# HudsonAlpha/rust-msbwt

Measured on AMD Instinct MI355X. Metric: k-mer count queries/sec (whole node), higher is better.
Workload: dtype u64

## Files before the change

rust-msbwt_amd/_build.py:

```python
import os
import subprocess
import sys

HERE = os.path.dirname(os.path.abspath(__file__))
CSRC = os.path.join(HERE, "csrc")
LIB = os.path.join(HERE, "libmsbwt_hip.so")
SOURCES = ["capi.cpp", "index_build.cpp", "query.cpp", "sources.cpp", "spectrum.cpp", "produce.cpp", "multi_device.cpp", "kernels.hip", "lanes.hip", "lanes_tier.hip", "lanes_wide.hip", "lanes_xwide.hip", "extend.hip", "sparse_table.hip", "device_build.hip", "pair_index.hip", "gather.hip", "order.hip", "run_build.hip", "reads_build.hip", "run_encode.hip", "merge.hip", "merge_many.hip", "source_index.hip", "spectrum.hip", "plane_index.cpp", "run_index.cpp", "npy_io.cpp", "rle_codec.cpp"]
HEADERS = ["handle.hpp", "index_build.hpp", "kernels.hpp", "lanes_kernel.hpp", "sparse_table.hpp", "sparse_build.hpp", "sparse_policy.hpp", "device_build.hpp", "pair_index.hpp", "gather.hpp", "order.hpp", "run_build.hpp", "reads_build.hpp", "run_encode.hpp", "merge.hpp", "merge_common.hpp", "source_index.hpp", "frontier.hpp", "spectrum.hpp", "rank_ops.hpp", "search_common.hpp", "host_pipeline.hpp", "plane_index.hpp", "run_index.hpp", "table_policy.hpp", "npy_io.hpp", "rle_codec.hpp", os.path.join("..", "..", "include", "msbwt_hip.h")]


def hipcc():
    for cand in (os.environ.get("HIPCC"), "/opt/rocm/bin/hipcc", "hipcc"):
        if cand and (os.path.isabs(cand) and os.path.exists(cand) or not os.path.isabs(cand)):
            return cand
    return "hipcc"


def stale():
    if not os.path.exists(LIB):
        return True
    t = os.path.getmtime(LIB)
    deps = [os.path.join(CSRC, f) for f in SOURCES + HEADERS] + [os.path.abspath(__file__)]
    return any(os.path.getmtime(d) > t for d in deps)


def build(force=False, verbose=False):
    if not force and not stale():
        return LIB
    from concurrent.futures import ThreadPoolExecutor

    objdir = os.path.join(HERE, "build")
    os.makedirs(objdir, exist_ok=True)
    common = ["-O3", "-std=c++17", "-fPIC", "-Wall", "-Wextra"]
    newest_header = max(os.path.getmtime(os.path.join(CSRC, f)) for f in HEADERS)
    newest_header = max(newest_header, os.path.getmtime(os.path.abspath(__file__)))

    def compile_one(src):
        obj = os.path.join(objdir, src + ".o")
        path = os.path.join(CSRC, src)
        if not force and os.path.exists(obj) and os.path.getmtime(obj) > max(os.path.getmtime(path), newest_header):
            return obj
# ... 21 lines not shown
```

rust-msbwt_amd/csrc/host_pipeline.hpp:

```cpp
#pragma once
#include <hip/hip_runtime_api.h>

#include <algorithm>
#include <condition_variable>
#include <cstdint>
#include <cstring>
#include <functional>
#include <memory>
#include <mutex>
#include <thread>
#include <vector>

namespace msbwt {

class CopyPool {
  public:
    explicit CopyPool(int threads) {
        for (int t = 0; t < threads; ++t) workers_.emplace_back([this, t] { loop(t); });
    }
    ~CopyPool() {
        {
            std::lock_guard<std::mutex> lock(mu_);
            stop_ = true;
        }
        wake_.notify_all();
        for (auto &w : workers_) w.join();
    }
    int threads() const { return int(workers_.size()); }

    void copy(void *dst, const void *src, size_t bytes) {
        if (bytes < (size_t(1) << 20) || workers_.empty()) {
            std::memcpy(dst, src, bytes);
            return;
        }
        std::unique_lock<std::mutex> lock(mu_);
        dst_ = static_cast<char *>(dst);
        src_ = static_cast<const char *>(src);
        bytes_ = bytes;
        pending_ = int(workers_.size());
        ++generation_;
        wake_.notify_all();
        done_.wait(lock, [this] { return pending_ == 0; });
    }

  private:
    void loop(int t) {
        uint64_t seen = 0;
        for (;;) {
            std::unique_lock<std::mutex> lock(mu_);
            wake_.wait(lock, [&] { return stop_ || generation_ != seen; });
            if (stop_) return;
            seen = generation_;
            const size_t n = workers_.size(), piece = (bytes_ / n + 63) / 64 * 64;
            const size_t lo = std::min(bytes_, piece * size_t(t)), hi = (size_t(t) + 1 == n) ? bytes_ : std::min(bytes_, lo + piece);
            char *d = dst_;
            const char *s = src_;
            lock.unlock();
            if (hi > lo) std::memcpy(d + lo, s + lo, hi - lo);
            lock.lock();
            if (--pending_ == 0) done_.notify_all();
        }
    }
    std::vector<std::thread> workers_;
    std::mutex mu_;
    std::condition_variable wake_, done_;
    bool stop_ = false;
    uint64_t generation_ = 0;
    int pending_ = 0;
    char *dst_ = nullptr;
    const char *src_ = nullptr;
    size_t bytes_ = 0;
};

struct HostArray {
    const void *in = nullptr;
    void *out = nullptr;
    size_t item_bytes = 0;
};

class HostPipeline {
  public:
    static constexpr int kSlots = 3;
    ~HostPipeline() { release(); }

    using Launch = std::function<hipError_t(size_t, size_t, void *const *, void *const *, hipStream_t)>;

    hipError_t run(size_t n, size_t chunk, const std::vector<HostArray> &ins, const std::vector<HostArray> &outs,
                   hipStream_t compute, const Launch &launch) {
        if (n == 0) return hipSuccess;
        chunk = std::max<size_t>(1, std::min(chunk, n));
        size_t in_bytes = 0, out_bytes = 0;
        std::vector<size_t> in_off, out_off;
        for (const HostArray &a : ins) { in_off.push_back(in_bytes); in_bytes += (chunk * a.item_bytes + 255) / 256 * 256; }
        for (const HostArray &a : outs) { out_off.push_back(out_bytes); out_bytes += (chunk * a.item_bytes + 255) / 256 * 256; }
        hipError_t e = ensure(in_bytes, out_bytes);
        if (e != hipSuccess) return e;
        if (!pool_) {
            const unsigned hw = std::thread::hardware_concurrency();
            pool_.reset(new CopyPool(int(std::max(2u, std::min(hw ? hw / 2 : 4u, 12u)))));
        }
        const size_t nchunks = (n + chunk - 1) / chunk;
        std::vector<void *> d_in(ins.size()), d_out(outs.size());
        auto finish = [&](size_t c) -> hipError_t {
            Slot &s = slots_[c % kSlots];
            hipError_t err = hipEventSynchronize(s.d2h);
            if (err != hipSuccess) return err;
            const size_t first = c * chunk, m = std::min(chunk, n - first);
            for (size_t a = 0; a < outs.size(); ++a)
                pool_->copy(static_cast<char *>(outs[a].out) + first * outs[a].item_bytes, s.h_out + out_off[a], m * outs[a].item_bytes);
            return hipSuccess;
        };
        for (size_t c = 0; c < nchunks + kSlots - 1; ++c) {
            if (c < nchunks) {
                Slot &s = slots_[c % kSlots];
                const size_t first = c * chunk, m = std::min(chunk, n - first);
                for (size_t a = 0; a < ins.size(); ++a)
                    pool_->copy(s.h_in + in_off[a], static_cast<const char *>(ins[a].in) + first * ins[a].item_bytes, m * ins[a].item_bytes);
                for (size_t a = 0; a < ins.size(); ++a) {
                    e = hipMemcpyAsync(s.d_in + in_off[a], s.h_in + in_off[a], m * ins[a].item_bytes, hipMemcpyHostToDevice, h2d_);
                    if (e != hipSuccess) return e;
                    d_in[a] = s.d_in + in_off[a];
                }
                for (size_t a = 0; a < outs.size(); ++a) d_out[a] = s.d_out + out_off[a];
                if ((e = hipEventRecord(s.up, h2d_)) != hipSuccess) return e;
                if ((e = hipStreamWaitEvent(compute, s.up, 0)) != hipSuccess) return e;
                if ((e = launch(first, m, d_in.data(), d_out.data(), compute)) != hipSuccess) return e;
                if ((e = hipEventRecord(s.done, compute)) != hipSuccess) return e;
                if ((e = hipStreamWaitEvent(d2h_, s.done, 0)) != hipSuccess) return e;
                for (size_t a = 0; a < outs.size(); ++a) {
                    e = hipMemcpyAsync(s.h_out + out_off[a], s.d_out + out_off[a], m * outs[a].item_bytes, hipMemcpyDeviceToHost, d2h_);
                    if (e != hipSuccess) return e;
                }
                if ((e = hipEventRecord(s.d2h, d2h_)) != hipSuccess) return e;
            }
            if (c >= size_t(kSlots - 1) && (e = finish(c - (kSlots - 1))) != hipSuccess) return e;
        }
        return hipSuccess;
    }

    void release() {
        for (Slot &s : slots_) {
            if (s.h_in) (void)hipHostFree(s.h_in);
            if (s.h_out) (void)hipHostFree(s.h_out);
            if (s.d_in) (void)hipFree(s.d_in);
            if (s.d_out) (void)hipFree(s.d_out);
            if (s.up) (void)hipEventDestroy(s.up);
            if (s.done) (void)hipEventDestroy(s.done);
            if (s.d2h) (void)hipEventDestroy(s.d2h);
            s = Slot{};
        }
        if (h2d_) (void)hipStreamDestroy(h2d_);
        if (d2h_) (void)hipStreamDestroy(d2h_);
        h2d_ = d2h_ = nullptr;
        in_cap_ = out_cap_ = 0;
    }

  private:
    struct Slot {
        char *h_in = nullptr, *h_out = nullptr, *d_in = nullptr, *d_out = nullptr;
        hipEvent_t up = nullptr, done = nullptr, d2h = nullptr;
    };

    hipError_t ensure(size_t in_bytes, size_t out_bytes) {
        hipError_t e;
        if (!h2d_ && (e = hipStreamCreateWithFlags(&h2d_, hipStreamNonBlocking)) != hipSuccess) return e;
        if (!d2h_ && (e = hipStreamCreateWithFlags(&d2h_, hipStreamNonBlocking)) != hipSuccess) return e;
        for (Slot &s : slots_) {
            if (!s.up && (e = hipEventCreateWithFlags(&s.up, hipEventDisableTiming)) != hipSuccess) return e;
            if (!s.done && (e = hipEventCreateWithFlags(&s.done, hipEventDisableTiming)) != hipSuccess) return e;
            if (!s.d2h && (e = hipEventCreateWithFlags(&s.d2h, hipEventDisableTiming)) != hipSuccess) return e;
        }
        if (in_bytes > in_cap_) {
            for (Slot &s : slots_) {
                if (s.h_in) (void)hipHostFree(s.h_in);
                if (s.d_in) (void)hipFree(s.d_in);
                s.h_in = s.d_in = nullptr;
            }
            in_cap_ = 0;
            for (Slot &s : slots_) {
                if ((e = hipHostMalloc(reinterpret_cast<void **>(&s.h_in), in_bytes, hipHostMallocDefault)) != hipSuccess) return e;
                if ((e = hipMalloc(reinterpret_cast<void **>(&s.d_in), in_bytes)) != hipSuccess) return e;
            }
            in_cap_ = in_bytes;
        }
        if (out_bytes > out_cap_) {
            for (Slot &s : slots_) {
                if (s.h_out) (void)hipHostFree(s.h_out);
                if (s.d_out) (void)hipFree(s.d_out);
                s.h_out = s.d_out = nullptr;
            }
            out_cap_ = 0;
            for (Slot &s : slots_) {
                if ((e = hipHostMalloc(reinterpret_cast<void **>(&s.h_out), out_bytes, hipHostMallocDefault)) != hipSuccess) return e;
                if ((e = hipMalloc(reinterpret_cast<void **>(&s.d_out), out_bytes)) != hipSuccess) return e;
            }
            out_cap_ = out_bytes;
        }
        return hipSuccess;
    }

    Slot slots_[kSlots];
    hipStream_t h2d_ = nullptr, d2h_ = nullptr;
    size_t in_cap_ = 0, out_cap_ = 0;
    std::unique_ptr<CopyPool> pool_;
};

}
```

rust-msbwt_amd/csrc/query.cpp:

```cpp
#include <algorithm>
#include <atomic>
#include <chrono>
#include <cstring>
#include <string>
#include <vector>

#include "gather.hpp"
#include "handle.hpp"
#include "order.hpp"

namespace {

constexpr size_t kMailQueries = 64, kMailKmerBytes = 4096;
constexpr size_t kMailDone = 0;
constexpr size_t kMailKmers = 64, kMailCounts = kMailKmers + kMailKmerBytes, kMailSyms = kMailCounts + 8 * kMailQueries,
                 kMailL = kMailSyms + 64, kMailH = kMailL + 8 * kMailQueries, kMailOutL = kMailH + 8 * kMailQueries,
                 kMailOutH = kMailOutL + 8 * kMailQueries, kMailBytes = kMailOutH + 8 * kMailQueries;

int ensure_mail(msbwt_rle *h) {
    if (int rc = ensure_runtime(h)) return rc;
    if (h->mail) return MSBWT_OK;
    void *host = nullptr, *dev = nullptr;
    HIP_TRY(h, hipHostMalloc(&host, kMailBytes, hipHostMallocMapped | hipHostMallocCoherent));
    const hipError_t e = hipHostGetDevicePointer(&dev, host, 0);
    if (e != hipSuccess) {
        (void)hipHostFree(host);
        return hip_fail(h, e, "hipHostGetDevicePointer");
    }
    std::memset(host, 0, kMailBytes);
    h->mail = static_cast<uint8_t *>(host);
    h->d_mail = static_cast<uint8_t *>(dev);
    return MSBWT_OK;
}

bool order_pays(msbwt_rle *h, const IndexView &v, size_t k, size_t n) {
    if (h->wanted_order <= 0 || v.block_format != kBlocksPlanes || v.pair_blocks == nullptr) return false;
    return k >= 12 && k <= 64 && n >= 4096 && n <= 0xFFFFFFFFull && lanes_serves(v, uint32_t(k));
}

bool ensure_order_scratch(msbwt_rle::TicketSlot &slot, size_t bytes) {
    if (bytes <= slot.order_bytes) return true;
    if (slot.order_scratch) (void)hipFree(slot.order_scratch);
// ... 106 lines not shown
            if (!ensure_range_scratch(slot, std::min(n, kBySourcePiece) * 2 * sizeof(uint64_t))) return hipErrorOutOfMemory;
            uint64_t *pairs = static_cast<uint64_t *>(slot.range_scratch);
            const SourceView sv = h->sources.view(v.total);
            hipError_t e = hipSuccess;
            for (size_t first = 0; first < n && e == hipSuccess; first += kBySourcePiece) {
                const size_t m = std::min(kBySourcePiece, n - first);
                e = launch_kmer_ranges(v, d_kmers + first * k, uint32_t(k), m, pairs, pairs + 1, 2u, h->d_flags + which, stream);
                if (e == hipSuccess) e = launch_range_sources(sv, pairs, pairs + 1, 2u, m, d_out + first * sv.n_sources, h->d_flags + which, stream);
            }
            return e;
        });
    });
}

int launch_sources_of_ranges(msbwt_rle *h, const uint64_t *d_l, const uint64_t *d_h, size_t n, uint64_t *d_out, hipStream_t stream, int which) {
    return timed_launch(h, stream, [&] { return launch_range_sources(h->sources.view(h->totals.total), d_l, d_h, 1u, n, d_out, h->d_flags + which, stream); });
}

int need_sources(msbwt_rle *h) { return h->sources.n_sources ? int(MSBWT_OK) : fail(h, MSBWT_ERR_NOT_LOADED, "no sources attached"); }

size_t by_source_chunk(const msbwt_rle *h) { return std::min(size_t(1) << 21, (size_t(96) << 20) / (h->sources.n_sources * sizeof(uint64_t))); }

int launch_read_kmers_locked(msbwt_rle *h, const void *d_reads, size_t read_len, size_t n_reads, size_t k,
                                    int ascii, void *d_out_fwd, void *d_out_rc, hipStream_t stream, int which) {
    return timed_with_tickets(h, stream, [&](const IndexView &v) {
        return launch_count_read_kmers(v, static_cast<const uint8_t *>(d_reads), uint32_t(read_len), n_reads, uint32_t(k), ascii != 0,
                                       static_cast<uint64_t *>(d_out_fwd), static_cast<uint64_t *>(d_out_rc), h->d_flags + which, stream);
    });
}

HostArray host_in(const void *p, size_t item_bytes) { return HostArray{p, nullptr, item_bytes}; }
HostArray host_out(void *p, size_t item_bytes) { return HostArray{nullptr, p, item_bytes}; }

template <class Launch>
int run_host_batch(msbwt_rle *h, size_t n, size_t chunk, const std::vector<HostArray> &ins, const std::vector<HostArray> &outs, const char *what,
                   Launch &&launch) {
    int launch_rc = MSBWT_OK;
    const hipError_t e = h->pipe.run(n, chunk, ins, outs, h->stream, [&](size_t, size_t m, void *const *d_in, void *const *d_out, hipStream_t stream) {
        launch_rc = launch(m, d_in, d_out, stream);
        return launch_rc ? hipErrorUnknown : hipSuccess;
    });
    if (launch_rc) return launch_rc;
    if (e != hipSuccess) return hip_fail(h, e, (std::string(what) + " pipeline").c_str());
    return status_of(h, h->stream, kHostFlags);
}

template <class Launch, class CopyOut>
int mailbox_call(msbwt_rle *h, IndexView &v, bool poll, Launch &&launch, CopyOut &&copy_out) {
    volatile uint64_t *done = reinterpret_cast<volatile uint64_t *>(h->mail + kMailDone);
    const uint64_t seq = ++h->mail_seq;
    if (poll) {
        v.done = reinterpret_cast<uint64_t *>(h->d_mail + kMailDone);
        v.done_seq = seq;
    }
    if (int rc = launch()) return rc;
    bool seen = false;
    if (poll) {
        const auto give_up = std::chrono::steady_clock::now() + std::chrono::milliseconds(2);
        for (unsigned spins = 0; !(seen = *done == seq); ++spins)
            if ((spins & 1023u) == 1023u && std::chrono::steady_clock::now() > give_up) break;
    }
    if (!seen) HIP_TRY(h, hipStreamSynchronize(h->stream));
    std::atomic_thread_fence(std::memory_order_acquire);
    return copy_out() ? status_of(h, h->stream, kHostFlags) : MSBWT_OK;
}

// ... 6 lines not shown
    Call c(ch);
    if (int rc = c.open(n && (!d_out_counts || (!d_kmers && k)), "null device pointer")) return rc;
    return launch_count(c.h, static_cast<const uint8_t *>(d_kmers), k, n, static_cast<uint64_t *>(d_out_counts),
                        static_cast<hipStream_t>(hip_stream), kDeviceFlags);
}

int msbwt_rle_count_kmers_packed_device(const msbwt_rle *ch, const void *d_kmers2bit, size_t k, size_t n, void *d_out_counts, void *hip_stream) {
    Call c(ch);
    if (int rc = c.open(n && (!d_out_counts || !d_kmers2bit), "null device pointer")) return rc;
    if (n == 0) return MSBWT_OK;
    return launch_count_2bit(c.h, static_cast<const uint64_t *>(d_kmers2bit), k, n, static_cast<uint64_t *>(d_out_counts), static_cast<hipStream_t>(hip_stream),
                             kDeviceFlags);
}

int msbwt_rle_count_kmers_packed(const msbwt_rle *ch, const uint64_t *kmers2bit, size_t k, size_t n, void *out_counts, int count_bits) {
    Call c(ch);
    const bool bad_k = k < 1 || k > 64 || (count_bits != 64 && count_bits != 32);
    if (int rc = c.open(bad_k || (n && (!out_counts || !kmers2bit)), bad_k ? "packed queries need 1 <= k <= 64 and 64- or 32-bit counts" : "null pointer")) return rc;
    if (n == 0) return MSBWT_OK;
    msbwt_rle *h = c.h;
    if (int rc = ensure_runtime(h)) return rc;
    const size_t words = k > 32 ? 2 : 1, chunk = size_t(1) << 22;
    if (int rc = count_bits == 32 ? ensure_stage(h, std::min(n, chunk) * sizeof(uint64_t)) : MSBWT_OK) return rc;
    return run_host_batch(h, n, chunk, {host_in(kmers2bit, words * sizeof(uint64_t))}, {host_out(out_counts, size_t(count_bits / 8))}, "count_kmers_packed",
                          [&](size_t m, void *const *d_in, void *const *d_out, hipStream_t stream) {
                              uint64_t *d_counts = count_bits == 64 ? static_cast<uint64_t *>(d_out[0]) : static_cast<uint64_t *>(h->d_stage);
                              if (int r = launch_count_2bit(h, static_cast<const uint64_t *>(d_in[0]), k, m, d_counts, stream, kHostFlags)) return r;
                              if (count_bits == 64) return int(MSBWT_OK);
                              const hipError_t e = launch_narrow_counts32(d_counts, static_cast<uint32_t *>(d_out[0]), m, h->d_flags + kHostFlags, stream);
                              return e == hipSuccess ? int(MSBWT_OK) : hip_fail(h, e, "count_kmers_packed pipeline");
                          });
}

int msbwt_kmers_pack_2bit(const uint8_t *kmers, size_t k, size_t n, uint64_t *out_words) {
    if (k < 1 || k > 64 || (n && (!kmers || !out_words))) return MSBWT_ERR_INVALID_ARG;
    const size_t words = k > 32 ? 2 : 1;
    for (size_t q = 0; q < n; ++q) {
        uint64_t w[2] = {0, 0};
        for (size_t t = 0; t < k; ++t) {
            const uint8_t s = kmers[q * k + k - 1 - t];
            if (s != 1 && s != 2 && s != 3 && s != 5) return MSBWT_ERR_INVALID_SYMBOL;
            w[t >> 5] |= uint64_t(s - 1 - (s >> 2)) << (2 * (t & 31));
        }
        for (size_t i = 0; i < words; ++i) out_words[q * words + i] = w[i];
    }
    return MSBWT_OK;
}

int msbwt_rle_set_batch_order(msbwt_rle *h, int mode) {
    if (!h || mode < -1 || mode > 1) return MSBWT_ERR_INVALID_ARG;
    return set_locked(h, h->wanted_order, mode);
}

int msbwt_rle_get_batch_order(const msbwt_rle *h) { return h ? h->wanted_order : 0; }

int msbwt_rle_batch_order_for(const msbwt_rle *ch, size_t k, size_t n) {
    if (!ch || !ch->loaded) return MSBWT_ERR_INVALID_ARG;
    Call c(ch);
    return order_pays(c.h, view_of(c.h), k, n) ? 1 : 0;
}

int msbwt_rle_constrain_ranges_device(const msbwt_rle *ch, const void *d_syms, const void *d_l, const void *d_h,
                                      size_t n, void *d_out_l, void *d_out_h, void *hip_stream) {
    Call c(ch);
    if (int rc = c.open(n && (!d_syms || !d_l || !d_h || !d_out_l || !d_out_h), "null device pointer")) return rc;
    msbwt_rle *h = c.h;
    HIP_TRY(h, launch_constrain_ranges(view_of(h), static_cast<const uint8_t *>(d_syms),
                                       static_cast<const uint64_t *>(d_l), static_cast<const uint64_t *>(d_h), n,
                                       static_cast<uint64_t *>(d_out_l), static_cast<uint64_t *>(d_out_h),
                                       h->d_flags + kDeviceFlags, static_cast<hipStream_t>(hip_stream)));
    return MSBWT_OK;
}

int msbwt_rle_count_read_kmers_device(const msbwt_rle *ch, const void *d_reads, size_t read_len, size_t n_reads,
                                      size_t k, int ascii, void *d_out_fwd, void *d_out_rc, void *hip_stream) {
    Call c(ch);
    const bool bad = k < 1 || k > 64 || k > read_len || read_len > 0xFFFFFFFFull || (!d_out_fwd && !d_out_rc) || (n_reads && !d_reads);
    if (int rc = c.open(bad, "count_read_kmers needs 1 <= k <= min(64, read_len) and an output")) return rc;
    return launch_read_kmers_locked(c.h, d_reads, read_len, n_reads, k, ascii, d_out_fwd, d_out_rc,
// ... 84 lines not shown
    msbwt_rle *h = c.h;
    if (!h) return MSBWT_ERR_INVALID_ARG;
    if (!h->d_flags) return MSBWT_OK;
    if (int rc = c.bind()) return rc;
    return status_of(h, static_cast<hipStream_t>(hip_stream), kDeviceFlags);
}

int msbwt_rle_count_kmers(const msbwt_rle *ch, const uint8_t *kmers, size_t k, size_t n, uint64_t *out_counts) {
    Call c(ch);
    if (int rc = c.open(n && (!out_counts || (!kmers && k)), "null pointer")) return rc;
    if (n == 0) return MSBWT_OK;
    msbwt_rle *h = c.h;
    if (n <= kMailQueries && n * k <= kMailKmerBytes) {
        if (int rc = ensure_mail(h)) return rc;
        const uint64_t *counts = reinterpret_cast<const uint64_t *>(h->mail + kMailCounts);
        if (!tier_launch_ok(h)) return hip_fail(h, hipErrorInvalidValue, "two-tier sparse table beside a direct table it cannot fall back to");
        IndexView v = view_of(h);
        const bool poll = k <= 0xFFFFFFFFull && lanes_serves(v, uint32_t(k));
        const bool inlined = poll && n == 1;
        if (k && !inlined) std::memcpy(h->mail + kMailKmers, kmers, n * k);
        auto launch = [&] {
            return launch_count_kmers(v, h->d_mail + kMailKmers, uint32_t(k), n, reinterpret_cast<uint64_t *>(h->d_mail + kMailCounts), h->d_flags + kHostFlags,
                                      h->stream, inlined ? kmers : nullptr);
        };
        return mailbox_call(h, v, poll, [&] { return timed_launch(h, h->stream, launch); }, [&] {
            bool flagged = false;
            for (size_t i = 0; i < n; ++i) {
                out_counts[i] = counts[i];
                flagged |= counts[i] == ~0ull;
            }
            return flagged;
        });
    }
    return run_host_batch(h, n, size_t(1) << 21, {host_in(kmers, k)}, {host_out(out_counts, sizeof(uint64_t))}, "count_kmers",
                          [&](size_t m, void *const *d_in, void *const *d_out, hipStream_t stream) {
                              return launch_count(h, static_cast<const uint8_t *>(d_in[0]), k, m, static_cast<uint64_t *>(d_out[0]), stream, kHostFlags);
                          });
}

int msbwt_rle_constrain_ranges(const msbwt_rle *ch, const uint8_t *syms, const uint64_t *l, const uint64_t *hh,
                               size_t n, uint64_t *out_l, uint64_t *out_h) {
    Call c(ch);
    if (int rc = c.open(n && (!syms || !l || !hh || !out_l || !out_h), "null pointer")) return rc;
    if (n == 0) return MSBWT_OK;
    msbwt_rle *h = c.h;
    if (n <= kMailQueries) {
        if (int rc = ensure_mail(h)) return rc;
        std::memcpy(h->mail + kMailSyms, syms, n);
        std::memcpy(h->mail + kMailL, l, n * sizeof(uint64_t));
        std::memcpy(h->mail + kMailH, hh, n * sizeof(uint64_t));
        IndexView v = view_of(h);
        const bool poll = n <= 8;
        auto launch = [&] {
            HIP_TRY(h, launch_constrain_ranges(v, h->d_mail + kMailSyms, reinterpret_cast<const uint64_t *>(h->d_mail + kMailL),
                                               reinterpret_cast<const uint64_t *>(h->d_mail + kMailH), n, reinterpret_cast<uint64_t *>(h->d_mail + kMailOutL),
                                               reinterpret_cast<uint64_t *>(h->d_mail + kMailOutH), h->d_flags + kHostFlags, h->stream));
            return int(MSBWT_OK);
        };
        return mailbox_call(h, v, poll, launch, [&] {
            const uint64_t *ol = reinterpret_cast<const uint64_t *>(h->mail + kMailOutL), *oh = reinterpret_cast<const uint64_t *>(h->mail + kMailOutH);
            bool flagged = false;
            for (size_t i = 0; i < n; ++i) {
                out_l[i] = ol[i];
                out_h[i] = oh[i];
                flagged |= ol[i] == ~0ull;
            }
            return flagged;
// ... 8 lines not shown
                              return e == hipSuccess ? int(MSBWT_OK) : hip_fail(h, e, "constrain_ranges pipeline");
                          });
}

int msbwt_rle_constrain_range(const msbwt_rle *h, uint8_t sym, uint64_t l, uint64_t hh, uint64_t *out_l,
                              uint64_t *out_h) {
    if (!out_l || !out_h) return MSBWT_ERR_INVALID_ARG;
    return msbwt_rle_constrain_ranges(h, &sym, &l, &hh, 1, out_l, out_h);
}

int msbwt_rle_count_kmer(const msbwt_rle *h, const uint8_t *kmer, size_t k, uint64_t *out_count) {
    if (!out_count) return MSBWT_ERR_INVALID_ARG;
    return msbwt_rle_count_kmers(h, kmer, k, 1, out_count);
}

int msbwt_rle_kmer_ranges_device(const msbwt_rle *ch, const void *d_kmers, size_t k, size_t n, void *d_out_l, void *d_out_h, void *hip_stream) {
    Call c(ch);
    if (int rc = c.open(n && (!d_out_l || !d_out_h || (!d_kmers && k)), "null device pointer")) return rc;
    return launch_ranges(c.h, static_cast<const uint8_t *>(d_kmers), k, n, static_cast<uint64_t *>(d_out_l), static_cast<uint64_t *>(d_out_h), 1u,
                         static_cast<hipStream_t>(hip_stream), kDeviceFlags);
}

int msbwt_rle_count_kmer_extensions_device(const msbwt_rle *ch, const void *d_kmers, size_t k, size_t n, void *d_out_counts, void *hip_stream) {
    Call c(ch);
    if (int rc = c.open(n && (!d_out_counts || (!d_kmers && k)), "null device pointer")) return rc;
    return launch_extensions(c.h, static_cast<const uint8_t *>(d_kmers), k, n, static_cast<uint64_t *>(d_out_counts), static_cast<hipStream_t>(hip_stream),
                             kDeviceFlags);
}

int msbwt_rle_kmer_ranges(const msbwt_rle *ch, const uint8_t *kmers, size_t k, size_t n, uint64_t *out_l, uint64_t *out_h) {
    Call c(ch);
    if (int rc = c.open(n && (!out_l || !out_h || (!kmers && k)), "null pointer")) return rc;
    if (n == 0) return MSBWT_OK;
    return run_host_batch(c.h, n, size_t(1) << 21, {host_in(kmers, k)}, {host_out(out_l, sizeof(uint64_t)), host_out(out_h, sizeof(uint64_t))}, "kmer_ranges",
                          [&](size_t m, void *const *d_in, void *const *d_out, hipStream_t stream) {
                              return launch_ranges(c.h, static_cast<const uint8_t *>(d_in[0]), k, m, static_cast<uint64_t *>(d_out[0]),
                                                   static_cast<uint64_t *>(d_out[1]), 1u, stream, kHostFlags);
                          });
}

int msbwt_rle_count_kmer_extensions(const msbwt_rle *ch, const uint8_t *kmers, size_t k, size_t n, uint64_t *out_counts) {
    Call c(ch);
    if (int rc = c.open(n && (!out_counts || (!kmers && k)), "null pointer")) return rc;
    if (n == 0) return MSBWT_OK;
    return run_host_batch(c.h, n, size_t(1) << 21, {host_in(kmers, k)}, {host_out(out_counts, 6 * sizeof(uint64_t))}, "count_kmer_extensions",
                          [&](size_t m, void *const *d_in, void *const *d_out, hipStream_t stream) {
                              return launch_extensions(c.h, static_cast<const uint8_t *>(d_in[0]), k, m, static_cast<uint64_t *>(d_out[0]), stream, kHostFlags);
                          });
}

int msbwt_rle_count_kmers_by_source_device(const msbwt_rle *ch, const void *d_kmers, size_t k, size_t n, void *d_out_counts, void *hip_stream) {
    Call c(ch);
    if (int rc = c.open()) return rc;
    if (int rc = need_sources(c.h)) return rc;
    if (n && (!d_out_counts || (!d_kmers && k))) return fail(c.h, MSBWT_ERR_INVALID_ARG, "null device pointer");
    if (n == 0) return MSBWT_OK;
    return launch_by_source(c.h, static_cast<const uint8_t *>(d_kmers), k, n, static_cast<uint64_t *>(d_out_counts), static_cast<hipStream_t>(hip_stream),
                            kDeviceFlags);
}

int msbwt_rle_count_kmers_by_source(const msbwt_rle *ch, const uint8_t *kmers, size_t k, size_t n, uint64_t *out_counts) {
    Call c(ch);
    if (int rc = c.open()) return rc;
    if (int rc = need_sources(c.h)) return rc;
    if (n && (!out_counts || (!kmers && k))) return fail(c.h, MSBWT_ERR_INVALID_ARG, "null pointer");
    if (n == 0) return MSBWT_OK;
    return run_host_batch(c.h, n, by_source_chunk(c.h), {host_in(kmers, k)}, {host_out(out_counts, c.h->sources.n_sources * sizeof(uint64_t))}, "count_kmers_by_source",
                          [&](size_t m, void *const *d_in, void *const *d_out, hipStream_t stream) {
                              return launch_by_source(c.h, static_cast<const uint8_t *>(d_in[0]), k, m, static_cast<uint64_t *>(d_out[0]), stream, kHostFlags);
                          });
}

int msbwt_rle_range_sources_device(const msbwt_rle *ch, const void *d_l, const void *d_h, size_t n, void *d_out_counts, void *hip_stream) {
    Call c(ch);
    if (int rc = c.open()) return rc;
    if (int rc = need_sources(c.h)) return rc;
    if (n && (!d_l || !d_h || !d_out_counts)) return fail(c.h, MSBWT_ERR_INVALID_ARG, "null device pointer");
    return launch_sources_of_ranges(c.h, static_cast<const uint64_t *>(d_l), static_cast<const uint64_t *>(d_h), n, static_cast<uint64_t *>(d_out_counts),
                                    static_cast<hipStream_t>(hip_stream), kDeviceFlags);
}

int msbwt_rle_range_sources(const msbwt_rle *ch, const uint64_t *l, const uint64_t *hh, size_t n, uint64_t *out_counts) {
    Call c(ch);
    if (int rc = c.open()) return rc;
    if (int rc = need_sources(c.h)) return rc;
    if (n && (!l || !hh || !out_counts)) return fail(c.h, MSBWT_ERR_INVALID_ARG, "null pointer");
    if (n == 0) return MSBWT_OK;
    return run_host_batch(c.h, n, by_source_chunk(c.h), {host_in(l, sizeof(uint64_t)), host_in(hh, sizeof(uint64_t))},
                          {host_out(out_counts, c.h->sources.n_sources * sizeof(uint64_t))}, "range_sources",
                          [&](size_t m, void *const *d_in, void *const *d_out, hipStream_t stream) {
                              return launch_sources_of_ranges(c.h, static_cast<const uint64_t *>(d_in[0]), static_cast<const uint64_t *>(d_in[1]), m,
                                                              static_cast<uint64_t *>(d_out[0]), stream, kHostFlags);
                          });
}

int msbwt_kmer_order_keys(const uint8_t *kmers, size_t k, size_t n, uint64_t *out_keys) {
    if (k < 1 || k > 0xFFFFFFFFull || (n && (!kmers || !out_keys))) return MSBWT_ERR_INVALID_ARG;
    order_keys_host(kmers, uint32_t(k), n, out_keys);
    return MSBWT_OK;
}
// ... 13 lines not shown
```

Baseline: 33.81 billion.

## Pack host k-mer queries to 2-bit words and expand them on device

Host-side k-mer query batches are now packed with AVX2/BMI2 into 2-bit words before the host-to-device copy, and a new device kernel expands them back to byte rows ahead of the search kernel. This cuts PCIe upload volume roughly fourfold for k between 9 and 64. The copy pool also gains spin-wait wakeups and a generic split job, and there are optional verbose stage timers. In exchange it adds host CPU packing work and an extra device kernel per chunk, and it falls back to a plain copy when a symbol is invalid.

```diff
diff --git a/rust-msbwt_amd/_build.py b/rust-msbwt_amd/_build.py
--- a/rust-msbwt_amd/_build.py
+++ b/rust-msbwt_amd/_build.py
@@ -5,8 +5,8 @@
 HERE = os.path.dirname(os.path.abspath(__file__))
 CSRC = os.path.join(HERE, "csrc")
 LIB = os.path.join(HERE, "libmsbwt_hip.so")
-SOURCES = ["capi.cpp", "index_build.cpp", "query.cpp", "sources.cpp", "spectrum.cpp", "produce.cpp", "multi_device.cpp", "kernels.hip", "lanes.hip", "lanes_tier.hip", "lanes_wide.hip", "lanes_xwide.hip", "extend.hip", "sparse_table.hip", "device_build.hip", "pair_index.hip", "gather.hip", "order.hip", "run_build.hip", "reads_build.hip", "run_encode.hip", "merge.hip", "merge_many.hip", "source_index.hip", "spectrum.hip", "plane_index.cpp", "run_index.cpp", "npy_io.cpp", "rle_codec.cpp"]
-HEADERS = ["handle.hpp", "index_build.hpp", "kernels.hpp", "lanes_kernel.hpp", "sparse_table.hpp", "sparse_build.hpp", "sparse_policy.hpp", "device_build.hpp", "pair_index.hpp", "gather.hpp", "order.hpp", "run_build.hpp", "reads_build.hpp", "run_encode.hpp", "merge.hpp", "merge_common.hpp", "source_index.hpp", "frontier.hpp", "spectrum.hpp", "rank_ops.hpp", "search_common.hpp", "host_pipeline.hpp", "plane_index.hpp", "run_index.hpp", "table_policy.hpp", "npy_io.hpp", "rle_codec.hpp", os.path.join("..", "..", "include", "msbwt_hip.h")]
+SOURCES = ["capi.cpp", "index_build.cpp", "query.cpp", "pack_stage.cpp", "sources.cpp", "spectrum.cpp", "produce.cpp", "multi_device.cpp", "kernels.hip", "lanes.hip", "lanes_tier.hip", "lanes_wide.hip", "lanes_xwide.hip", "extend.hip", "expand.hip", "sparse_table.hip", "device_build.hip", "pair_index.hip", "gather.hip", "order.hip", "run_build.hip", "reads_build.hip", "run_encode.hip", "merge.hip", "merge_many.hip", "source_index.hip", "spectrum.hip", "plane_index.cpp", "run_index.cpp", "npy_io.cpp", "rle_codec.cpp"]
+HEADERS = ["handle.hpp", "index_build.hpp", "kernels.hpp", "lanes_kernel.hpp", "sparse_table.hpp", "sparse_build.hpp", "sparse_policy.hpp", "device_build.hpp", "pair_index.hpp", "gather.hpp", "order.hpp", "run_build.hpp", "reads_build.hpp", "run_encode.hpp", "merge.hpp", "merge_common.hpp", "source_index.hpp", "frontier.hpp", "spectrum.hpp", "rank_ops.hpp", "search_common.hpp", "host_pipeline.hpp", "pack_stage.hpp", "expand.hpp", "plane_index.hpp", "run_index.hpp", "table_policy.hpp", "npy_io.hpp", "rle_codec.hpp", os.path.join("..", "..", "include", "msbwt_hip.h")]
 
 
 def hipcc():
diff --git a/rust-msbwt_amd/csrc/expand.hip b/rust-msbwt_amd/csrc/expand.hip
--- /dev/null
+++ b/rust-msbwt_amd/csrc/expand.hip
@@ -0,0 +1,58 @@
+#include <hip/hip_runtime.h>
+
+#include <algorithm>
+
+#include "expand.hpp"
+
+namespace msbwt {
+
+namespace {
+
+constexpr uint32_t kExpandThreads = 256, kExpandBytes = 16;
+
+__global__ __launch_bounds__(kExpandThreads) void k_expand_rows(const uint64_t *__restrict__ packed, uint32_t k, uint64_t bytes, uint8_t *__restrict__ rows) {
+    const uint32_t words = k > 32u ? 2u : 1u;
+    const uint64_t groups = (bytes + kExpandBytes - 1) / kExpandBytes, stride = uint64_t(gridDim.x) * blockDim.x;
+    for (uint64_t g = uint64_t(blockIdx.x) * blockDim.x + threadIdx.x; g < groups; g += stride) {
+        const uint64_t b0 = g * kExpandBytes;
+        const uint32_t len = uint32_t(std::min<uint64_t>(kExpandBytes, bytes - b0));
+        uint64_t q = b0 / k;
+        uint32_t j = uint32_t(b0 - q * k);
+        uint32_t t = k - 1u - j;
+        uint64_t w = packed[q * words + (t >> 5)];
+        uint32_t out[kExpandBytes / 4] = {0, 0, 0, 0};
+#pragma unroll
+        for (uint32_t i = 0; i < kExpandBytes; ++i) {
+            if (i < len) {
+                const uint32_t c = uint32_t(w >> (2u * (t & 31u))) & 3u;
+                out[i >> 2] |= (c + 1u + (c == 3u ? 1u : 0u)) << (8u * (i & 3u));
+                if (t == 0u) {
+                    ++q;
+                    t = k - 1u;
+                    if (i + 1u < len) w = packed[q * words + (t >> 5)];
+                } else {
+                    --t;
+                    if ((t & 31u) == 31u) w = packed[q * words];
+                }
+            }
+        }
+        if (len == kExpandBytes) {
+            *reinterpret_cast<uint4 *>(rows + b0) = make_uint4(out[0], out[1], out[2], out[3]);
+        } else {
+            for (uint32_t i = 0; i < len; ++i) rows[b0 + i] = uint8_t(out[i >> 2] >> (8u * (i & 3u)));
+        }
+    }
+}
+
+}
+
+hipError_t launch_expand_rows(const uint64_t *d_packed, uint32_t k, uint64_t n, uint8_t *d_rows, hipStream_t stream) {
+    if (n == 0) return hipSuccess;
+    if (k < 1u || k > 64u || (reinterpret_cast<uintptr_t>(d_rows) & 15u) || (reinterpret_cast<uintptr_t>(d_packed) & 7u)) return hipErrorInvalidValue;
+    const uint64_t bytes = n * k, groups = (bytes + kExpandBytes - 1) / kExpandBytes;
+    const uint64_t blocks = std::min<uint64_t>((groups + kExpandThreads - 1) / kExpandThreads, 256 * 32);
+    hipLaunchKernelGGL(k_expand_rows, dim3(uint32_t(blocks)), dim3(kExpandThreads), 0, stream, d_packed, k, bytes, d_rows);
+    return hipGetLastError();
+}
+
+}
diff --git a/rust-msbwt_amd/csrc/expand.hpp b/rust-msbwt_amd/csrc/expand.hpp
--- /dev/null
+++ b/rust-msbwt_amd/csrc/expand.hpp
@@ -0,0 +1,10 @@
+#pragma once
+#include <hip/hip_runtime_api.h>
+
+#include <cstdint>
+
+namespace msbwt {
+
+hipError_t launch_expand_rows(const uint64_t *d_packed, uint32_t k, uint64_t n, uint8_t *d_rows, hipStream_t stream);
+
+}
diff --git a/rust-msbwt_amd/csrc/host_pipeline.hpp b/rust-msbwt_amd/csrc/host_pipeline.hpp
--- a/rust-msbwt_amd/csrc/host_pipeline.hpp
+++ b/rust-msbwt_amd/csrc/host_pipeline.hpp
@@ -2,8 +2,12 @@
 #include <hip/hip_runtime_api.h>
 
 #include <algorithm>
+#include <atomic>
+#include <chrono>
 #include <condition_variable>
 #include <cstdint>
+#include <cstdio>
+#include <cstdlib>
 #include <cstring>
 #include <functional>
 #include <memory>
@@ -15,67 +19,107 @@
 
 class CopyPool {
   public:
-    explicit CopyPool(int threads) {
+    using Job = std::function<void(size_t, size_t)>;
+    explicit CopyPool(int threads) : count_(size_t(std::max(threads, 0))) {
         for (int t = 0; t < threads; ++t) workers_.emplace_back([this, t] { loop(t); });
     }
     ~CopyPool() {
         {
             std::lock_guard<std::mutex> lock(mu_);
-            stop_ = true;
+            stop_.store(true, std::memory_order_release);
         }
         wake_.notify_all();
         for (auto &w : workers_) w.join();
     }
-    int threads() const { return int(workers_.size()); }
+    int threads() const { return int(count_); }
 
     void copy(void *dst, const void *src, size_t bytes) {
-        if (bytes < (size_t(1) << 20) || workers_.empty()) {
+        if (bytes < (size_t(1) << 20) || count_ == 0) {
             std::memcpy(dst, src, bytes);
             return;
         }
+        char *d = static_cast<char *>(dst);
+        const char *s = static_cast<const char *>(src);
+        split(bytes, 64, [d, s](size_t lo, size_t hi) { std::memcpy(d + lo, s + lo, hi - lo); });
+    }
+
+    void split(size_t items, size_t grain, const Job &fn) {
+        if (count_ == 0) {
+            fn(0, items);
+            return;
+        }
+        fn_ = &fn;
+        items_ = items;
+        grain_ = std::max<size_t>(1, grain);
+        pending_.store(int(count_), std::memory_order_relaxed);
+        {
+            std::lock_guard<std::mutex> lock(mu_);
+            generation_.fetch_add(1, std::memory_order_release);
+        }
+        wake_.notify_all();
+        if (watch([this] { return pending_.load(std::memory_order_acquire) == 0; }, kCallerWatch)) return;
         std::unique_lock<std::mutex> lock(mu_);
-        dst_ = static_cast<char *>(dst);
-        src_ = static_cast<const char *>(src);
-        bytes_ = bytes;
-        pending_ = int(workers_.size());
-        ++generation_;
-        wake_.notify_all();
-        done_.wait(lock, [this] { return pending_ == 0; });
+        done_.wait(lock, [this] { return pending_.load(std::memory_order_acquire) == 0; });
     }
 
   private:
-    void loop(int t) {
+    static constexpr int kWorkerWatch = 200, kCallerWatch = 50;
+
+    template <class Ready>
+    static bool watch(Ready &&ready, int us) {
+        const auto until = std::chrono::steady_clock::now() + std::chrono::microseconds(us);
+        for (unsigned spins = 0;; ++spins) {
+            if (ready()) return true;
+#if defined(__x86_64__) || defined(__i386__)
+            __builtin_ia32_pause();
+#else
+            std::this_thread::yield();
+#endif
+            if ((spins & 63u) == 63u && std::chrono::steady_clock::now() > until) return false;
+        }
+    }
+
+    void loop(size_t t) {
         uint64_t seen = 0;
+        auto news = [&] { return stop_.load(std::memory_order_acquire) || generation_.load(std::memory_order_acquire) != seen; };
         for (;;) {
-            std::unique_lock<std::mutex> lock(mu_);
-            wake_.wait(lock, [&] { return stop_ || generation_ != seen; });
-            if (stop_) return;
-            seen = generation_;
-            const size_t n = workers_.size(), piece = (bytes_ / n + 63) / 64 * 64;
-            const size_t lo = std::min(bytes_, piece * size_t(t)), hi = (size_t(t) + 1 == n) ? bytes_ : std::min(bytes_, lo + piece);
-            char *d = dst_;
-            const char *s = src_;
-            lock.unlock();
-            if (hi > lo) std::memcpy(d + lo, s + lo, hi - lo);
-            lock.lock();
-            if (--pending_ == 0) done_.notify_all();
-        }
-    }
+            if (!watch(news, kWorkerWatch)) {
+                std::unique_lock<std::mutex> lock(mu_);
+                wake_.wait(lock, news);
+            }
+            if (stop_.load(std::memory_order_acquire)) return;
+            seen = generation_.load(std::memory_order_acquire);
+            const size_t piece = (items_ / count_ + grain_ - 1) / grain_ * grain_;
+            const size_t lo = std::min(items_, piece * t), hi = (t + 1 == count_) ? items_ : std::min(items_, lo + piece);
+            if (hi > lo) (*fn_)(lo, hi);
+            if (pending_.fetch_sub(1, std::memory_order_acq_rel) == 1) {
+                { std::lock_guard<std::mutex> lock(mu_); }
+                done_.notify_one();
+            }
+        }
+    }
+    const size_t count_;
     std::vector<std::thread> workers_;
     std::mutex mu_;
     std::condition_variable wake_, done_;
-    bool stop_ = false;
-    uint64_t generation_ = 0;
-    int pending_ = 0;
-    char *dst_ = nullptr;
-    const char *src_ = nullptr;
-    size_t bytes_ = 0;
+    std::atomic<bool> stop_{false};
+    std::atomic<uint64_t> generation_{0};
+    std::atomic<int> pending_{0};
+    const Job *fn_ = nullptr;
+    size_t items_ = 0, grain_ = 1;
+};
+
+struct Stager {
+    size_t item_bytes = 0;
+    std::function<bool(void *dst, const void *src, size_t items)> pack;
+    std::function<hipError_t(void *d_items, const void *d_compact, size_t m, hipStream_t stream)> expand;
 };
 
 struct HostArray {
     const void *in = nullptr;
     void *out = nullptr;
     size_t item_bytes = 0;
+    const Stager *stager = nullptr;
 };
 
 class HostPipeline {
@@ -93,37 +137,63 @@
         std::vector<size_t> in_off, out_off;
         for (const HostArray &a : ins) { in_off.push_back(in_bytes); in_bytes += (chunk * a.item_bytes + 255) / 256 * 256; }
         for (const HostArray &a : outs) { out_off.push_back(out_bytes); out_bytes += (chunk * a.item_bytes + 255) / 256 * 256; }
-        hipError_t e = ensure(in_bytes, out_bytes);
+        size_t compact_bytes = 0;
+        std::vector<size_t> compact_off;
+        for (const HostArray &a : ins) { compact_off.push_back(compact_bytes); compact_bytes += a.stager ? (chunk * a.stager->item_bytes + 255) / 256 * 256 : 0; }
+        hipError_t e = ensure(in_bytes, out_bytes, compact_bytes);
         if (e != hipSuccess) return e;
         if (!pool_) {
             const unsigned hw = std::thread::hardware_concurrency();
             pool_.reset(new CopyPool(int(std::max(2u, std::min(hw ? hw / 2 : 4u, 12u)))));
         }
         const size_t nchunks = (n + chunk - 1) / chunk;
+        const bool verbose = std::getenv("MSBWT_VERBOSE") != nullptr;
+        double spent[4] = {0, 0, 0, 0};
+        auto now = [] { return std::chrono::steady_clock::now(); };
+        auto lap = [&](int what, std::chrono::steady_clock::time_point &t) {
+            if (!verbose) return;
+            const auto t1 = now();
+            spent[what] += std::chrono::duration<double>(t1 - t).count();
+            t = t1;
+        };
         std::vector<void *> d_in(ins.size()), d_out(outs.size());
+        std::vector<char> compact(ins.size());
         auto finish = [&](size_t c) -> hipError_t {
             Slot &s = slots_[c % kSlots];
+            auto t = now();
             hipError_t err = hipEventSynchronize(s.d2h);
+            lap(2, t);
             if (err != hipSuccess) return err;
             const size_t first = c * chunk, m = std::min(chunk, n - first);
             for (size_t a = 0; a < outs.size(); ++a)
                 pool_->copy(static_cast<char *>(outs[a].out) + first * outs[a].item_bytes, s.h_out + out_off[a], m * outs[a].item_bytes);
+            lap(3, t);
             return hipSuccess;
         };
         for (size_t c = 0; c < nchunks + kSlots - 1; ++c) {
             if (c < nchunks) {
                 Slot &s = slots_[c % kSlots];
                 const size_t first = c * chunk, m = std::min(chunk, n - first);
-                for (size_t a = 0; a < ins.size(); ++a)
-                    pool_->copy(s.h_in + in_off[a], static_cast<const char *>(ins[a].in) + first * ins[a].item_bytes, m * ins[a].item_bytes);
+                auto t = now();
                 for (size_t a = 0; a < ins.size(); ++a) {
-                    e = hipMemcpyAsync(s.d_in + in_off[a], s.h_in + in_off[a], m * ins[a].item_bytes, hipMemcpyHostToDevice, h2d_);
+                    const char *src = static_cast<const char *>(ins[a].in) + first * ins[a].item_bytes;
+                    compact[a] = ins[a].stager && stage_compact(*ins[a].stager, s.h_in + in_off[a], src, ins[a].item_bytes, m);
+                    if (!compact[a]) pool_->copy(s.h_in + in_off[a], src, m * ins[a].item_bytes);
+                }
+                lap(0, t);
+                for (size_t a = 0; a < ins.size(); ++a) {
+                    if (compact[a])
+                        e = hipMemcpyAsync(s.d_compact + compact_off[a], s.h_in + in_off[a], m * ins[a].stager->item_bytes, hipMemcpyHostToDevice, h2d_);
+                    else
+                        e = hipMemcpyAsync(s.d_in + in_off[a], s.h_in + in_off[a], m * ins[a].item_bytes, hipMemcpyHostToDevice, h2d_);
                     if (e != hipSuccess) return e;
                     d_in[a] = s.d_in + in_off[a];
                 }
                 for (size_t a = 0; a < outs.size(); ++a) d_out[a] = s.d_out + out_off[a];
                 if ((e = hipEventRecord(s.up, h2d_)) != hipSuccess) return e;
                 if ((e = hipStreamWaitEvent(compute, s.up, 0)) != hipSuccess) return e;
+                for (size_t a = 0; a < ins.size(); ++a)
+                    if (compact[a] && (e = ins[a].stager->expand(d_in[a], s.d_compact + compact_off[a], m, compute)) != hipSuccess) return e;
                 if ((e = launch(first, m, d_in.data(), d_out.data(), compute)) != hipSuccess) return e;
                 if ((e = hipEventRecord(s.done, compute)) != hipSuccess) return e;
                 if ((e = hipStreamWaitEvent(d2h_, s.done, 0)) != hipSuccess) return e;
@@ -132,9 +202,13 @@
                     if (e != hipSuccess) return e;
                 }
                 if ((e = hipEventRecord(s.d2h, d2h_)) != hipSuccess) return e;
+                lap(1, t);
             }
             if (c >= size_t(kSlots - 1) && (e = finish(c - (kSlots - 1))) != hipSuccess) return e;
         }
+        if (verbose)
+            std::fprintf(stderr, "[msbwt] host pipeline: %zu items in %zu chunks; staging %.3f ms, enqueueing %.3f, waiting for the device %.3f, results back %.3f\n", n,
+                         nchunks, spent[0] * 1e3, spent[1] * 1e3, spent[2] * 1e3, spent[3] * 1e3);
         return hipSuccess;
     }
 
@@ -144,6 +218,7 @@
             if (s.h_out) (void)hipHostFree(s.h_out);
             if (s.d_in) (void)hipFree(s.d_in);
             if (s.d_out) (void)hipFree(s.d_out);
+            if (s.d_compact) (void)hipFree(s.d_compact);
             if (s.up) (void)hipEventDestroy(s.up);
             if (s.done) (void)hipEventDestroy(s.done);
             if (s.d2h) (void)hipEventDestroy(s.d2h);
@@ -152,16 +227,25 @@
         if (h2d_) (void)hipStreamDestroy(h2d_);
         if (d2h_) (void)hipStreamDestroy(d2h_);
         h2d_ = d2h_ = nullptr;
-        in_cap_ = out_cap_ = 0;
+        in_cap_ = out_cap_ = compact_cap_ = 0;
     }
 
   private:
     struct Slot {
-        char *h_in = nullptr, *h_out = nullptr, *d_in = nullptr, *d_out = nullptr;
+        char *h_in = nullptr, *h_out = nullptr, *d_in = nullptr, *d_out = nullptr, *d_compact = nullptr;
         hipEvent_t up = nullptr, done = nullptr, d2h = nullptr;
     };
 
-    hipError_t ensure(size_t in_bytes, size_t out_bytes) {
+    bool stage_compact(const Stager &st, char *dst, const char *src, size_t item_bytes, size_t m) {
+        if (m * item_bytes < (size_t(1) << 20)) return st.pack(dst, src, m);
+        std::atomic<bool> ok{true};
+        pool_->split(m, 64, [&](size_t lo, size_t hi) {
+            if (ok.load(std::memory_order_relaxed) && !st.pack(dst + lo * st.item_bytes, src + lo * item_bytes, hi - lo)) ok.store(false, std::memory_order_relaxed);
+        });
+        return ok.load();
+    }
+
+    hipError_t ensure(size_t in_bytes, size_t out_bytes, size_t compact_bytes) {
         hipError_t e;
         if (!h2d_ && (e = hipStreamCreateWithFlags(&h2d_, hipStreamNonBlocking)) != hipSuccess) return e;
         if (!d2h_ && (e = hipStreamCreateWithFlags(&d2h_, hipStreamNonBlocking)) != hipSuccess) return e;
@@ -196,12 +280,22 @@
             }
             out_cap_ = out_bytes;
         }
+        if (compact_bytes > compact_cap_) {
+            for (Slot &s : slots_) {
+                if (s.d_compact) (void)hipFree(s.d_compact);
+                s.d_compact = nullptr;
+            }
+            compact_cap_ = 0;
+            for (Slot &s : slots_)
+                if ((e = hipMalloc(reinterpret_cast<void **>(&s.d_compact), compact_bytes)) != hipSuccess) return e;
+            compact_cap_ = compact_bytes;
+        }
         return hipSuccess;
     }
 
     Slot slots_[kSlots];
     hipStream_t h2d_ = nullptr, d2h_ = nullptr;
-    size_t in_cap_ = 0, out_cap_ = 0;
+    size_t in_cap_ = 0, out_cap_ = 0, compact_cap_ = 0;
     std::unique_ptr<CopyPool> pool_;
 };
 
diff --git a/rust-msbwt_amd/csrc/pack_stage.cpp b/rust-msbwt_amd/csrc/pack_stage.cpp
--- /dev/null
+++ b/rust-msbwt_amd/csrc/pack_stage.cpp
@@ -0,0 +1,104 @@
+#include "pack_stage.hpp"
+
+#include <cstring>
+
+#if defined(__x86_64__) && (defined(__GNUC__) || defined(__clang__))
+#define MSBWT_PACK_STAGE_X86 1
+#include <immintrin.h>
+#endif
+
+namespace msbwt {
+
+namespace {
+
+bool pack_scalar(const uint8_t *kmers, size_t k, size_t n, uint64_t *out_words) {
+    const size_t words = k > 32 ? 2 : 1;
+    for (size_t q = 0; q < n; ++q) {
+        uint64_t w[2] = {0, 0};
+        for (size_t t = 0; t < k; ++t) {
+            const uint8_t s = kmers[q * k + k - 1 - t];
+            if (s != 1 && s != 2 && s != 3 && s != 5) return false;
+            w[t >> 5] |= uint64_t(s - 1 - (s >> 2)) << (2 * (t & 31));
+        }
+        for (size_t i = 0; i < words; ++i) out_words[q * words + i] = w[i];
+    }
+    return true;
+}
+
+#ifdef MSBWT_PACK_STAGE_X86
+#define MSBWT_PACK_TARGET __attribute__((target("avx2,bmi2")))
+
+alignas(32) const uint8_t kTakeMask[64] = {255, 255, 255, 255, 255, 255, 255, 255, 255, 255, 255, 255, 255, 255, 255, 255,
+                                           255, 255, 255, 255, 255, 255, 255, 255, 255, 255, 255, 255, 255, 255, 255, 255};
+
+MSBWT_PACK_TARGET inline uint64_t pack32(__m256i v, unsigned take, __m256i &bad) {
+    const __m256i table = _mm256_setr_epi8(0, 4, 5, 6, 0, 7, 0, 0, 0, 0, 0, 0, 0, 0, 0, 0, 0, 4, 5, 6, 0, 7, 0, 0, 0, 0, 0, 0, 0, 0, 0, 0);
+    const __m256i reverse = _mm256_setr_epi8(15, 14, 13, 12, 11, 10, 9, 8, 7, 6, 5, 4, 3, 2, 1, 0, 15, 14, 13, 12, 11, 10, 9, 8, 7, 6, 5, 4, 3, 2, 1, 0);
+    const __m256i coded = _mm256_shuffle_epi8(table, v);
+    const __m256i wrong = _mm256_or_si256(_mm256_andnot_si256(coded, _mm256_set1_epi8(4)), _mm256_and_si256(v, _mm256_set1_epi8(char(0xF0))));
+    const __m256i taken = _mm256_loadu_si256(reinterpret_cast<const __m256i *>(kTakeMask + 32 - take));
+    bad = _mm256_or_si256(bad, _mm256_and_si256(wrong, taken));
+    const __m256i r = _mm256_shuffle_epi8(coded, reverse);
+    const uint64_t two = 0x0303030303030303ull;
+    const uint64_t all = _pext_u64(uint64_t(_mm256_extract_epi64(r, 2)), two) | _pext_u64(uint64_t(_mm256_extract_epi64(r, 3)), two) << 16 |
+                         _pext_u64(uint64_t(_mm256_extract_epi64(r, 0)), two) << 32 | _pext_u64(uint64_t(_mm256_extract_epi64(r, 1)), two) << 48;
+    return all >> (2u * (32u - take));
+}
+
+MSBWT_PACK_TARGET bool pack_avx2(const uint8_t *kmers, size_t k, size_t n, uint64_t *out_words) {
+    constexpr size_t kLook = 1024;
+    __m256i bad = _mm256_setzero_si256();
+    if (k > 32) {
+        const unsigned rest = unsigned(k - 32);
+        for (size_t q0 = 0; q0 < n; q0 += kLook) {
+            const size_t q1 = q0 + kLook < n ? q0 + kLook : n;
+            for (size_t q = q0; q < q1; ++q) {
+                const uint8_t *p = kmers + q * k;
+                out_words[2 * q] = pack32(_mm256_loadu_si256(reinterpret_cast<const __m256i *>(p + rest)), 32u, bad);
+                out_words[2 * q + 1] = pack32(_mm256_loadu_si256(reinterpret_cast<const __m256i *>(p)), rest, bad);
+            }
+            if (!_mm256_testz_si256(bad, bad)) return false;
+        }
+        return true;
+    }
+    const size_t bytes = n * k, whole = bytes >= 32 ? (bytes - 32) / k + 1 : 0;
+    for (size_t q0 = 0; q0 < whole; q0 += kLook) {
+        const size_t q1 = q0 + kLook < whole ? q0 + kLook : whole;
+        for (size_t q = q0; q < q1; ++q) out_words[q] = pack32(_mm256_loadu_si256(reinterpret_cast<const __m256i *>(kmers + q * k)), unsigned(k), bad);
+        if (!_mm256_testz_si256(bad, bad)) return false;
+    }
+    for (size_t q = whole; q < n; ++q) {
+        alignas(32) uint8_t row[32] = {};
+        std::memcpy(row, kmers + q * k, k);
+        out_words[q] = pack32(_mm256_load_si256(reinterpret_cast<const __m256i *>(row)), unsigned(k), bad);
+    }
+    return _mm256_testz_si256(bad, bad) != 0;
+}
+#endif
+
+}
+
+bool pack_stage_fast() {
+#ifdef MSBWT_PACK_STAGE_X86
+    static const bool fast = __builtin_cpu_supports("avx2") && __builtin_cpu_supports("bmi2");
+    return fast;
+#else
+    return false;
+#endif
+}
+
+bool pack_stage(const uint8_t *kmers, size_t k, size_t n, uint64_t *out_words) {
+#ifdef MSBWT_PACK_STAGE_X86
+    if (pack_stage_fast()) return pack_avx2(kmers, k, n, out_words);
+#endif
+    return pack_scalar(kmers, k, n, out_words);
+}
+
+}
+
+extern "C" int msbwt_pack_stage_2bit(const uint8_t *kmers, size_t k, size_t n, uint64_t *out_words, int force_scalar) {
+    if (k < 1 || k > 64 || (n && (!kmers || !out_words))) return -1;
+    return (force_scalar ? msbwt::pack_scalar(kmers, k, n, out_words) : msbwt::pack_stage(kmers, k, n, out_words)) ? 1 : 0;
+}
+
+extern "C" int msbwt_pack_stage_is_fast(void) { return msbwt::pack_stage_fast() ? 1 : 0; }
diff --git a/rust-msbwt_amd/csrc/pack_stage.hpp b/rust-msbwt_amd/csrc/pack_stage.hpp
--- /dev/null
+++ b/rust-msbwt_amd/csrc/pack_stage.hpp
@@ -0,0 +1,16 @@
+#pragma once
+#include <cstddef>
+#include <cstdint>
+
+namespace msbwt {
+
+bool pack_stage_fast();
+
+bool pack_stage(const uint8_t *kmers, size_t k, size_t n, uint64_t *out_words);
+
+}
+
+extern "C" int msbwt_pack_stage_2bit(const uint8_t *kmers, size_t k, size_t n, uint64_t *out_words, int force_scalar);
+extern "C" int msbwt_pack_stage_is_fast(void);
+
+extern "C" uint64_t msbwt_host_pack_queries(void);
diff --git a/rust-msbwt_amd/csrc/query.cpp b/rust-msbwt_amd/csrc/query.cpp
--- a/rust-msbwt_amd/csrc/query.cpp
+++ b/rust-msbwt_amd/csrc/query.cpp
@@ -5,9 +5,11 @@
 #include <string>
 #include <vector>
 
+#include "expand.hpp"
 #include "gather.hpp"
 #include "handle.hpp"
 #include "order.hpp"
+#include "pack_stage.hpp"
 
 namespace {
 
@@ -180,6 +182,30 @@
 HostArray host_in(const void *p, size_t item_bytes) { return HostArray{p, nullptr, item_bytes}; }
 HostArray host_out(void *p, size_t item_bytes) { return HostArray{nullptr, p, item_bytes}; }
 
+std::atomic<uint64_t> g_queries_sent_packed{0};
+
+class KmerInput {
+  public:
+    KmerInput(const uint8_t *kmers, size_t k) : kmers_(kmers), k_(k) {
+        const char *env = std::getenv("MSBWT_HOST_PACK");
+        if (k < 9 || k > 64 || !pack_stage_fast() || (env && env[0] == '0' && env[1] == 0)) return;
+        packed_ = true;
+        stager_.item_bytes = (k > 32 ? 2 : 1) * sizeof(uint64_t);
+        stager_.pack = [k](void *dst, const void *src, size_t items) { return pack_stage(static_cast<const uint8_t *>(src), k, items, static_cast<uint64_t *>(dst)); };
+        stager_.expand = [k](void *d_rows, const void *d_words, size_t m, hipStream_t stream) {
+            g_queries_sent_packed.fetch_add(m, std::memory_order_relaxed);
+            return launch_expand_rows(static_cast<const uint64_t *>(d_words), uint32_t(k), m, static_cast<uint8_t *>(d_rows), stream);
+        };
+    }
+    HostArray in() const { return HostArray{kmers_, nullptr, k_, packed_ ? &stager_ : nullptr}; }
+
+  private:
+    const uint8_t *kmers_;
+    size_t k_;
+    bool packed_ = false;
+    Stager stager_;
+};
+
 template <class Launch>
 int run_host_batch(msbwt_rle *h, size_t n, size_t chunk, const std::vector<HostArray> &ins, const std::vector<HostArray> &outs, const char *what,
                    Launch &&launch) {
@@ -252,19 +278,11 @@
                           });
 }
 
+uint64_t msbwt_host_pack_queries(void) { return g_queries_sent_packed.load(std::memory_order_relaxed); }
+
 int msbwt_kmers_pack_2bit(const uint8_t *kmers, size_t k, size_t n, uint64_t *out_words) {
     if (k < 1 || k > 64 || (n && (!kmers || !out_words))) return MSBWT_ERR_INVALID_ARG;
-    const size_t words = k > 32 ? 2 : 1;
-    for (size_t q = 0; q < n; ++q) {
-        uint64_t w[2] = {0, 0};
-        for (size_t t = 0; t < k; ++t) {
-            const uint8_t s = kmers[q * k + k - 1 - t];
-            if (s != 1 && s != 2 && s != 3 && s != 5) return MSBWT_ERR_INVALID_SYMBOL;
-            w[t >> 5] |= uint64_t(s - 1 - (s >> 2)) << (2 * (t & 31));
-        }
-        for (size_t i = 0; i < words; ++i) out_words[q * words + i] = w[i];
-    }
-    return MSBWT_OK;
+    return pack_stage(kmers, k, n, out_words) ? MSBWT_OK : MSBWT_ERR_INVALID_SYMBOL;
 }
 
 int msbwt_rle_set_batch_order(msbwt_rle *h, int mode) {
@@ -415,7 +433,8 @@
             return flagged;
         });
     }
-    return run_host_batch(h, n, size_t(1) << 21, {host_in(kmers, k)}, {host_out(out_counts, sizeof(uint64_t))}, "count_kmers",
+    const KmerInput queries(kmers, k);
+    return run_host_batch(h, n, size_t(1) << 21, {queries.in()}, {host_out(out_counts, sizeof(uint64_t))}, "count_kmers",
                           [&](size_t m, void *const *d_in, void *const *d_out, hipStream_t stream) {
                               return launch_count(h, static_cast<const uint8_t *>(d_in[0]), k, m, static_cast<uint64_t *>(d_out[0]), stream, kHostFlags);
                           });
@@ -490,7 +509,8 @@
     Call c(ch);
     if (int rc = c.open(n && (!out_l || !out_h || (!kmers && k)), "null pointer")) return rc;
     if (n == 0) return MSBWT_OK;
-    return run_host_batch(c.h, n, size_t(1) << 21, {host_in(kmers, k)}, {host_out(out_l, sizeof(uint64_t)), host_out(out_h, sizeof(uint64_t))}, "kmer_ranges",
+    const KmerInput queries(kmers, k);
+    return run_host_batch(c.h, n, size_t(1) << 21, {queries.in()}, {host_out(out_l, sizeof(uint64_t)), host_out(out_h, sizeof(uint64_t))}, "kmer_ranges",
                           [&](size_t m, void *const *d_in, void *const *d_out, hipStream_t stream) {
                               return launch_ranges(c.h, static_cast<const uint8_t *>(d_in[0]), k, m, static_cast<uint64_t *>(d_out[0]),
                                                    static_cast<uint64_t *>(d_out[1]), 1u, stream, kHostFlags);
@@ -501,7 +521,8 @@
     Call c(ch);
     if (int rc = c.open(n && (!out_counts || (!kmers && k)), "null pointer")) return rc;
     if (n == 0) return MSBWT_OK;
-    return run_host_batch(c.h, n, size_t(1) << 21, {host_in(kmers, k)}, {host_out(out_counts, 6 * sizeof(uint64_t))}, "count_kmer_extensions",
+    const KmerInput queries(kmers, k);
+    return run_host_batch(c.h, n, size_t(1) << 21, {queries.in()}, {host_out(out_counts, 6 * sizeof(uint64_t))}, "count_kmer_extensions",
                           [&](size_t m, void *const *d_in, void *const *d_out, hipStream_t stream) {
                               return launch_extensions(c.h, static_cast<const uint8_t *>(d_in[0]), k, m, static_cast<uint64_t *>(d_out[0]), stream, kHostFlags);
                           });
@@ -523,7 +544,8 @@
     if (int rc = need_sources(c.h)) return rc;
     if (n && (!out_counts || (!kmers && k))) return fail(c.h, MSBWT_ERR_INVALID_ARG, "null pointer");
     if (n == 0) return MSBWT_OK;
-    return run_host_batch(c.h, n, by_source_chunk(c.h), {host_in(kmers, k)}, {host_out(out_counts, c.h->sources.n_sources * sizeof(uint64_t))}, "count_kmers_by_source",
+    const KmerInput queries(kmers, k);
+    return run_host_batch(c.h, n, by_source_chunk(c.h), {queries.in()}, {host_out(out_counts, c.h->sources.n_sources * sizeof(uint64_t))}, "count_kmers_by_source",
                           [&](size_t m, void *const *d_in, void *const *d_out, hipStream_t stream) {
                               return launch_by_source(c.h, static_cast<const uint8_t *>(d_in[0]), k, m, static_cast<uint64_t *>(d_out[0]), stream, kHostFlags);
                           });
```

Measured after the change: 32.27 billion. 4.6% lower.
